# glennhickey/teHmm

Measured on AMD Instinct MI355X. Metric: genome positions/sec (Viterbi+posterior), 35 states x 10 tracks, higher is better.
Workload: dtype f64

## Files before the change

tehmm_amd/csrc/tehmm_fused.hip.h:

```cpp
#pragma once
#include "tehmm_lane.hip.h"

namespace tehmm {

template <int NT>
struct FusedGeom {
  static constexpr int KS = NT / 4;
  static constexpr int KSP = ((KS + 1) + 1) & ~1;
  static constexpr int RT = (NT + 15) / 16;
  static constexpr int SLICE_B = KSP * 8;
  static constexpr int ROW_D = 4 * KSP;
  static constexpr int ROW_D_LDS = 4 * KSP + 2;
};

#ifndef TEHMM_FUSED_2W
#define TEHMM_FUSED_2W 36
#endif
#define TEHMM_FUSED_BLKW 24
#ifndef TEHMM_FUSED_NSLOT_CAP
#define TEHMM_FUSED_NSLOT_CAP 64
#endif

struct FusedTab {
  const unsigned long long *rixx;
  const double *ptab;
  const double *ptab_lds;
  int FKW;
  int SB, NB;
  int K, n_glb;
  int lds_rows;
  double normalize;
};

template <int NT>
__device__ __forceinline__ void fused_load_lds(const double *lds, int row, int kq, double (&x)[FusedGeom<NT>::KSP]) {
  using G = FusedGeom<NT>;
  lds_cd2 *p = (lds_cd2 *)(size_t)((unsigned)(size_t)(__attribute__((address_space(3))) const double *)lds +
                                   (unsigned)(row * (G::ROW_D_LDS * 8) + kq * G::SLICE_B));
#pragma unroll
  for (int i = 0; i < G::KSP / 2; ++i) {
    const d2v v = p[i];
    x[2 * i] = v.x;
    x[2 * i + 1] = v.y;
  }
}
template <int NT>
__device__ __forceinline__ void fused_load_glb(const double *tab, int row, int kq, double (&x)[FusedGeom<NT>::KSP]) {
  using G = FusedGeom<NT>;
  const double2 *p = (const double2 *)(tab + ((int64_t)row * 4 + kq) * G::KSP);
#pragma unroll
  for (int i = 0; i < G::KSP / 2; ++i) {
    const double2 v = p[i];
    x[2 * i] = v.x;
    x[2 * i + 1] = v.y;
  }
}

__device__ __forceinline__ double item_sum4(double t) {
  const unsigned lo = __double2loint(t), hi = __double2hiint(t);
  const auto a = __builtin_amdgcn_permlane32_swap(lo, lo, false, false);
  const auto b = __builtin_amdgcn_permlane32_swap(hi, hi, false, false);
  const double t1 = __hiloint2double((int)b[0], (int)a[0]) + __hiloint2double((int)b[1], (int)a[1]);
  const unsigned lo1 = __double2loint(t1), hi1 = __double2hiint(t1);
  const auto c = __builtin_amdgcn_permlane16_swap(lo1, lo1, false, false);
  const auto d = __builtin_amdgcn_permlane16_swap(hi1, hi1, false, false);
  return __hiloint2double((int)d[0], (int)c[0]) + __hiloint2double((int)d[1], (int)c[1]);
}
__device__ __forceinline__ double item_max4(double t) {
  const unsigned lo = __double2loint(t), hi = __double2hiint(t);
  const auto a = __builtin_amdgcn_permlane32_swap(lo, lo, false, false);
  const auto b = __builtin_amdgcn_permlane32_swap(hi, hi, false, false);
  const double t1 = fmax(__hiloint2double((int)b[0], (int)a[0]), __hiloint2double((int)b[1], (int)a[1]));
  const unsigned lo1 = __double2loint(t1), hi1 = __double2hiint(t1);
  const auto c = __builtin_amdgcn_permlane16_swap(lo1, lo1, false, false);
  const auto d = __builtin_amdgcn_permlane16_swap(hi1, hi1, false, false);
  return fmax(__hiloint2double((int)d[0], (int)c[0]), __hiloint2double((int)d[1], (int)c[1]));
}

typedef unsigned int fused_u4 __attribute__((ext_vector_type(4)));
struct IndexWindow {
  const fused_u4 *src;
  unsigned lds_base;
  int lane, dir, NB;
  int cur = -1;
  fused_u4 r0, r1, r2;
  bool inflight = false;

  __device__ __forceinline__ void request(int blk) {
    if (blk < 0 || blk >= NB) { inflight = false; return; }
    const fused_u4 *p = src + (int64_t)blk * 192 + lane * 3;
    r0 = p[0];
    r1 = p[1];
    r2 = p[2];
    inflight = true;
  }
  __device__ __forceinline__ void commit(int blk) {
    typedef __attribute__((address_space(3))) fused_u4 lds_u4;
    lds_u4 *d = (lds_u4 *)(size_t)(lds_base + (unsigned)((blk & 1) * 3072 + lane * 48));
    d[0] = r0;
    d[1] = r1;
    d[2] = r2;
    cur = blk;
  }
  __device__ __forceinline__ void start(int blk) {
    request(blk);
    commit(blk);
    request(blk + dir);
  }
  __device__ __forceinline__ void need(int blk) {
    if (blk != cur) {
      commit(blk);
      request(blk + dir);
    }
  }
  __device__ __forceinline__ unsigned word_addr(int blk, int r, int FKW, int w) const {
    return lds_base + (unsigned)((blk & 1) * 3072 + ((r * FKW + w) * 16 + (lane & 15)) * 8);
  }
};
__device__ __forceinline__ unsigned long long lds_read_u64(unsigned addr) {
  typedef __attribute__((address_space(3))) const unsigned long long lds_cu64;
  return *(lds_cu64 *)(size_t)addr;
}

template <int NT, bool LOGDOM>
struct EmisStream {
  using G = FusedGeom<NT>;
  static constexpr int NSLOT = G::KS < TEHMM_FUSED_NSLOT_CAP ? G::KS : TEHMM_FUSED_NSLOT_CAP;
  static constexpr int NGS = NSLOT > 1 ? 2 : 1;
  static constexpr int GF = NSLOT >= 8 ? 4 : NSLOT / 2;
  const FusedTab &ft;
  const double *lds;
  IndexWindow &win;
  const int kq;
  unsigned wbase = 0;
  double q[G::KS];
  double sc = 0.0;
  double xa[G::KSP];
  double xc[G::KSP];
  unsigned long long wcur = 0;

  __device__ __forceinline__ EmisStream(const FusedTab &ft_, const double *lds_, IndexWindow &win_, int kq_)
      : ft(ft_), lds(lds_), win(win_), kq(kq_) {}
  static __device__ __forceinline__ int entry(unsigned long long w, int i) { return (int)((w >> (16 * (i & 3))) & 0xffffull); }
  __device__ __forceinline__ unsigned long long word(int w) const { return lds_read_u64(wbase + (unsigned)w * 128u); }
  __device__ __forceinline__ void fold(const double (&x)[G::KSP]) {
#pragma unroll
    for (int s = 0; s < G::KS; ++s) q[s] = LOGDOM ? q[s] + x[s] : q[s] * x[s];
    if (!LOGDOM) sc += x[G::KS];
  }
  __device__ __forceinline__ void glb_request(int i) { fused_load_glb<NT>(ft.ptab, entry(word(i >> 2), i), kq, xa); }
  __device__ __forceinline__ void begin(int e) {
    const int blk = e / ft.SB, r = e - blk * ft.SB;
    win.need(blk);
    wbase = win.word_addr(blk, r, ft.FKW, 0);
#pragma unroll
    for (int s = 0; s < G::KS; ++s) q[s] = LOGDOM ? 0.0 : 1.0;
    sc = 0.0;
    glb_request(0);
    wcur = word(ft.n_glb >> 2);
  }
  __device__ __forceinline__ void slot(int k) {
    if (k >= NSLOT) return;
    const int il = ft.n_glb + k;
    if (k > 0) fold(xc);
    if (k == GF && NSLOT > 1) {
      fold(xa);
      glb_request(1);
    }
    fused_load_lds<NT>(lds, entry(wcur, il), kq, xc);
    if (k + 1 < NSLOT) wcur = word((il + 1) >> 2);
  }
  __device__ __forceinline__ void finish(int N, double (&qo)[G::KS], double &ms) {
    fold(xc);
    fold(xa);
    for (int i = NGS; i < ft.n_glb; ++i) {
      glb_request(i);
      fold(xa);
    }
    for (int il = ft.n_glb + NSLOT; il < ft.K; ++il) {
      fused_load_lds<NT>(lds, entry(word(il >> 2), il), kq, xc);
      fold(xc);
    }
    if (LOGDOM) {
      double m = -INFINITY;
#pragma unroll
      for (int s = 0; s < G::KS; ++s) {
        q[s] *= ft.normalize;
        m = fmax(m, kq + 4 * s < N ? q[s] : -INFINITY);
      }
      m = item_max4(m);
      const bool good = m > -1e20;
#pragma unroll
      for (int s = 0; s < G::KS; ++s) qo[s] = (good && kq + 4 * s < N) ? exp_nonpos(q[s] - m) : 0.0;
      ms = good ? m : 0.0;
    } else {
#pragma unroll
      for (int s = 0; s < G::KS; ++s) qo[s] = q[s];
      ms = sc;
    }
  }
};

template <int NT>
__host__ __device__ inline size_t fused_lds_bytes(int lds_rows, bool post_tiles) {
  return (size_t)lds_rows * FusedGeom<NT>::ROW_D_LDS * 8 + 4 * 2 * 3072 + (post_tiles ? 4 * (16 * NT * 8 + 128) : 0);
}
template <int NT>
__device__ __forceinline__ void fused_stage(const FusedTab &ft, double *lds) {
  const int n = ft.lds_rows * FusedGeom<NT>::ROW_D_LDS;
  for (int i = threadIdx.x; i < n; i += blockDim.x) lds[i] = ft.ptab_lds[i];
}

struct FusedOrder {
  int K, n_glb, FKW, KP, SB, NB, Wu;
  int zero_glb, zero_lds;
  unsigned char order[TEHMM_MAX_TRACKS];
  int base[TEHMM_MAX_TRACKS];
  int cnt[TEHMM_MAX_TRACKS];
};
__global__ __launch_bounds__(256) void k_fused_rowindex(IntervalTab iv, LaneGeom lg, FusedOrder fo, const uint8_t *obs,
                                                        unsigned long long *rixx) {
  const int E = fo.NB * fo.SB;
  const int64_t n = (int64_t)lg.n_groups * 4 * E * 16;
  const int per_blk = 16 * fo.SB;
  for (int64_t idx = blockIdx.x * (int64_t)blockDim.x + threadIdx.x; idx < n; idx += (int64_t)gridDim.x * blockDim.x) {
    const int64_t tb = idx / per_blk;
    const int rem = (int)(idx - tb * per_blk);
    const int i16 = rem / fo.SB;
    const int e = (int)(tb % fo.NB) * fo.SB + (rem - i16 * fo.SB);
    const int64_t tile = tb / fo.NB;
    const int64_t item = tile * 16 + i16;
    const bool valid = item < lg.n_items;
    const int id = valid ? lg.item_iv[item] : 0;
    const int64_t T = iv.len[id];
    int64_t t = (valid ? lg.item_t0[item] : 0) - fo.Wu + e;
    t = t < 0 ? 0 : (t >= T ? T - 1 : t);
    const uint8_t *orow = obs + (iv.pos0[id] + (T > 0 ? t : 0)) * fo.KP;
    const int blk = e / fo.SB, r = e - blk * fo.SB;
    unsigned long long *dst = rixx + ((tile * fo.NB + blk) * TEHMM_FUSED_BLKW + (int64_t)r * fo.FKW) * 16 + i16;
    for (int w = 0; w < fo.FKW; ++w) {
      unsigned long long word = 0;
      for (int b = 0; b < 4; ++b) {
        const int i = 4 * w + b;
        int v = 0;
        if (i < fo.K) {
          const int sym = orow[fo.order[i]];
          v = sym < fo.cnt[i] ? fo.base[i] + sym : (i < fo.n_glb ? fo.zero_glb : fo.zero_lds);
        }
        word |= (unsigned long long)(v & 0xffff) << (16 * b);
      }
      dst[(int64_t)w * 16] = word;
    }
  }
}

template <int NT, bool LOGDOM>
__global__ __launch_bounds__(256) __attribute__((amdgpu_waves_per_eu(NT <= TEHMM_FUSED_2W ? 2 : 1, NT <= TEHMM_FUSED_2W ? 2 : 1)))
void k_fused_fwd(IntervalTab iv, FusedTab ft, LaneGeom lg, int N, int CS, int Wu,
                 const double *__restrict__ tab , float *al32, double *chkf, double *pre,
                 double *end, double *slog32) {
  using G = FusedGeom<NT>;
  constexpr int KS = G::KS, RT = G::RT;
  extern __shared__ double fused_lds[];
  fused_stage<NT>(ft, fused_lds);
  __syncthreads();
  const int lane = threadIdx.x & 63;
  const int tile = blockIdx.x * 4 + (threadIdx.x >> 6);
  if (tile >= lg.n_groups * 4) return;
  const int L = lg.L;
  const int kq = lane >> 4;
  const int64_t item = (int64_t)tile * 16 + (lane & 15);
  const bool valid = item < lg.n_items;
  const int id = valid ? lg.item_iv[item] : 0;
  const int64_t t0 = valid ? lg.item_t0[item] : 0;
  const int64_t T = iv.len[id];
  const int64_t ct0 = (t0 / CS) * CS;
  const bool run = valid && ct0 + CS <= T && ct0 > 0;
  if (!__any(run)) return;
  double tf[RT][KS];
#pragma unroll
  for (int rt = 0; rt < RT; ++rt) {
#pragma unroll
    for (int s = 0; s < KS; ++s) {
      const int j = 16 * rt + (lane & 15), k = 4 * s + kq;
      tf[rt][s] = (j < NT) ? tab[k * NT + j] : 0.0;
    }
  }
  double v[KS];
#pragma unroll
  for (int s = 0; s < KS; ++s) v[s] = (kq + 4 * s < N) ? 1.0 / (double)N : 0.0;
  double slog = 0.0;
  auto vec_out = [&](double *dst) {
    const int64_t po = ((((item >> 6) * NT) + kq) << 6) + (item & 63);
#pragma unroll
    for (int s = 0; s < KS; ++s) dst[po + ((int64_t)(4 * s) << 6)] = v[s];
  };
  const double qnan = __longlong_as_double(0x7ff8000000000000LL);
  IndexWindow win;
  win.src = (const fused_u4 *)ft.rixx + (int64_t)tile * ft.NB * 192;
  win.lds_base = (unsigned)(size_t)(__attribute__((address_space(3))) const double *)fused_lds +
                 (unsigned)(ft.lds_rows * G::ROW_D_LDS * 8 + (threadIdx.x >> 6) * 2 * 3072);
  win.lane = lane;
  win.dir = 1;
  win.NB = ft.NB;
  win.start(0);
  double q[KS], ms;
  EmisStream<NT, LOGDOM> es(ft, fused_lds, win, kq);
  es.begin(0);
#pragma unroll
  for (int k = 0; k < KS; ++k) es.slot(k);
  es.finish(N, q, ms);
  const int E1 = ft.NB * ft.SB - 1;
  es.begin(min(1, E1));
  {
    float2 *ar = (float2 *)al32 + al32_index<NT>(lg, item, 0, kq) / 2;
#pragma unroll
    for (int p = 0; p < (KS + 1) / 2; ++p) ar[(int64_t)p * 64] = make_float2(0.f, 0.f);
  }
#ifdef TEHMM_STAMPS
  unsigned long long stq[4] = {0, 0, 0, 0}, stt = stamp_now();
#define FST(i) do { const unsigned long long n_ = stamp_now(); stq[i] += n_ - stt; stt = n_; } while (0)
#else
#define FST(i)
#endif
  for (int s = -Wu; s < L; ++s) {
    if (s == 0) {
      if (run) vec_out(pre);
      slog = 0.0;
    }
    FST(3);
    lane_d4 acc[RT];
#pragma unroll
    for (int rt = 0; rt < RT; ++rt) acc[rt] = (lane_d4){0.0, 0.0, 0.0, 0.0};
#pragma unroll
    for (int k = 0; k < KS; ++k) {
#pragma unroll
      for (int rt = 0; rt < RT; ++rt) acc[rt] = __builtin_amdgcn_mfma_f64_16x16x4f64(tf[rt][k], v[k], acc[rt], 0, 0, 0);
      es.slot(k);
      __builtin_amdgcn_sched_barrier(0);
    }
    FST(0);
    double qn[KS], msn = 0.0;
    es.finish(N, qn, msn);
    FST(1);
    double a[KS];
    double t = 0.0;
#pragma unroll
    for (int k = 0; k < KS; ++k) {
      a[k] = acc[k >> 2][k & 3] * q[k];
      t += a[k];
    }
    t = item_sum4(t);
    const int e = ((__double2hiint(t) >> 20) & 0x7ff) - 1022;
    const bool okrow = t > 1e-280 && t < INFINITY;
    const double scale = okrow ? __hiloint2double((1023 - e) << 20, 0) : qnan;
#pragma unroll
    for (int k = 0; k < KS; ++k) v[k] = a[k] * scale;
    slog += (double)e * 0.6931471805599453 + ms;
#pragma unroll
    for (int k = 0; k < KS; ++k) q[k] = qn[k];
    const double ms_now = ms;
    ms = msn;
    (void)ms_now;
    es.begin(min(s + 2 + Wu, E1));
    FST(2);
    {
      float2 *ar = (float2 *)al32 + al32_index<NT>(lg, item, s < 0 ? 0 : s, kq) / 2;
#pragma unroll
      for (int p = 0; p < (KS + 1) / 2; ++p)
        ar[(int64_t)p * 64] = run ? make_float2((float)v[2 * p], 2 * p + 1 < KS ? (float)v[2 * p + 1] : 0.f)
                                  : make_float2(0.f, 0.f);
    }
    if (s >= 0 && run) {
      if ((s & 31) == 31) {
        if (kq == 0) slog32[item * (L / 32) + (s >> 5)] = slog;
        if ((s & 63) == 31) {
          double *cr = chkf + (item * (L / 64) + (s >> 6)) * NT + kq;
#pragma unroll
          for (int k = 0; k < KS; ++k) cr[4 * k] = v[k];
        }
      }
    }
  }
  if (run) vec_out(end);
#ifdef TEHMM_STAMPS
  if (lane == 0 && blockIdx.x < 4096)
    for (int i = 0; i < 4; ++i) g_stamps[(blockIdx.x * 4 + (threadIdx.x >> 6)) * 4 + i] = stq[i];
#endif
#undef FST
}

template <int NT, bool LOGDOM, bool EPS, bool ESTEP = false>
__global__ __launch_bounds__(256) __attribute__((amdgpu_waves_per_eu(NT <= TEHMM_FUSED_2W ? 2 : 1, NT <= TEHMM_FUSED_2W ? 2 : 1)))
void k_fused_bwd(IntervalTab iv, FusedTab ft, LaneGeom lg, int N, int CS, int Wu,
                 const double *__restrict__ tab , const float *__restrict__ al32,
                 double *post, double *pre, double *end, double *chk, float *gam32 = nullptr, float *wz32 = nullptr,
                 double *sink = nullptr ) {
  using G = FusedGeom<NT>;
  constexpr int KS = G::KS, RT = G::RT;
  extern __shared__ double fused_lds[];
  fused_stage<NT>(ft, fused_lds);
  __syncthreads();
  const int lane = threadIdx.x & 63;
  const int tile = blockIdx.x * 4 + (threadIdx.x >> 6);
  if (tile >= lg.n_groups * 4) return;
  const int L = lg.L;
  const int kq = lane >> 4;
  const int64_t item = (int64_t)tile * 16 + (lane & 15);
  const bool valid = item < lg.n_items;
  const int id = valid ? lg.item_iv[item] : 0;
  const int64_t t0 = valid ? lg.item_t0[item] : 0;
  const int64_t T = iv.len[id];
  const int64_t ct0 = (t0 / CS) * CS;
  const bool run = valid && ct0 + CS <= T && ct0 + CS < T;
  if (!__any(run)) return;
  const int wu = !run ? 0 : (int)min((int64_t)Wu, T - (t0 + L));
  double tf[RT][KS];
#pragma unroll
  for (int rt = 0; rt < RT; ++rt) {
#pragma unroll
    for (int s = 0; s < KS; ++s) {
      const int j = 16 * rt + (lane & 15), k = 4 * s + kq;
      tf[rt][s] = (j < NT) ? tab[j * NT + k] : 0.0;
    }
  }
  double v[KS];
#pragma unroll
  for (int s = 0; s < KS; ++s) v[s] = 0.0;
  const int64_t prow0 = (iv.out0[id] + t0) * N;
  auto vec_out = [&](double *dst) {
    const int64_t po = ((((item >> 6) * NT) + kq) << 6) + (item & 63);
#pragma unroll
    for (int s = 0; s < KS; ++s) dst[po + ((int64_t)(4 * s) << 6)] = v[s];
  };
  const double eps = 1.1920928955078125e-07;
  const double inv_epsden = 1.0 / (1.0 + (double)N * eps);
  const double qnan = __longlong_as_double(0x7ff8000000000000LL);
  const int top = L + wu - 1;
  IndexWindow win;
  win.src = (const fused_u4 *)ft.rixx + (int64_t)tile * ft.NB * 192;
  win.lds_base = (unsigned)(size_t)(__attribute__((address_space(3))) const double *)fused_lds +
                 (unsigned)(ft.lds_rows * G::ROW_D_LDS * 8 + (threadIdx.x >> 6) * 2 * 3072);
  win.lane = lane;
  win.dir = -1;
  win.NB = ft.NB;
  win.start((L + 2 * Wu - 1) / ft.SB);
  typedef __attribute__((address_space(3))) double lds_f64;
  typedef __attribute__((address_space(3))) long long lds_i64;
  const unsigned ptile = (unsigned)(size_t)(__attribute__((address_space(3))) const double *)fused_lds +
                         (unsigned)(ft.lds_rows * G::ROW_D_LDS * 8 + 4 * 2 * 3072 + (threadIdx.x >> 6) * (16 * NT * 8 + 128));
  const unsigned pinfo = ptile + 16 * NT * 8;
  if (!ESTEP && kq == 0) *(lds_i64 *)(size_t)(pinfo + (lane & 15) * 8) = run ? (long long)prow0 : -1ll;
  double q[KS], ms;
  EmisStream<NT, LOGDOM> es(ft, fused_lds, win, kq);
  es.begin(L + 2 * Wu - 1);
#pragma unroll
  for (int k = 0; k < KS; ++k) es.slot(k);
  es.finish(N, q, ms);
  es.begin(max(L + 2 * Wu - 2, 0));
#ifdef TEHMM_STAMPS
  unsigned long long stq[4] = {0, 0, 0, 0}, stt = stamp_now();
#define FST(i) do { const unsigned long long n_ = stamp_now(); stq[i] += n_ - stt; stt = n_; } while (0)
#else
#define FST(i)
#endif
  for (int s = L + Wu - 1; s >= 0; --s) {
    if (s == L - 1 && run) vec_out(pre);
    FST(3);
    lane_d4 acc[RT];
#pragma unroll
    for (int rt = 0; rt < RT; ++rt) acc[rt] = (lane_d4){0.0, 0.0, 0.0, 0.0};
    float2 alp[(KS + 1) / 2];
    {
      const float2 *ar = (const float2 *)al32 + al32_index<NT>(lg, item, s < L ? s : L - 1, kq) / 2;
#pragma unroll
      for (int p = 0; p < (KS + 1) / 2; ++p) alp[p] = ar[(int64_t)p * 64];
    }
#pragma unroll
    for (int k = 0; k < KS; ++k) {
#pragma unroll
      for (int rt = 0; rt < RT; ++rt) acc[rt] = __builtin_amdgcn_mfma_f64_16x16x4f64(tf[rt][k], v[k], acc[rt], 0, 0, 0);
      es.slot(k);
      __builtin_amdgcn_sched_barrier(0);
    }
    FST(0);
#pragma unroll
    for (int p = 0; p < (KS + 1) / 2; ++p) asm volatile("" : "+v"(alp[p].x), "+v"(alp[p].y));
#pragma unroll
    for (int p = 0; p < (KS + 1) / 2; ++p) alp[p] = run ? alp[p] : make_float2(0.f, 0.f);
    double qn[KS], msn = 0.0;
    es.finish(N, qn, msn);
    FST(1);
    double t = 0.0;
#pragma unroll
    for (int k = 0; k < KS; ++k) t += acc[k >> 2][k & 3];
    t = item_sum4(t);
    const int e = ((__double2hiint(t) >> 20) & 0x7ff) - 1022;
    double bt[KS];
    const bool okrow = (s >= L && s >= top) || (t > 0.0 && t < INFINITY);
    const double scale = okrow ? __hiloint2double((1023 - e) << 20, 0) : qnan;
#pragma unroll
    for (int k = 0; k < KS; ++k) {
      bt[k] = acc[k >> 2][k & 3] * scale;
      if (s >= L && s == top) bt[k] = kq + 4 * k < N ? 1.0 : 0.0;
    }
    double g[KS];
    float wzf[ESTEP ? KS : 1];
#pragma unroll
    for (int k = 0; k < KS; ++k) g[k] = 0.0;
#pragma unroll
    for (int k = 0; k < (ESTEP ? KS : 1); ++k) wzf[k] = 0.f;
    if (s < L) {
      double gt = 0.0;
#pragma unroll
      for (int k = 0; k < KS; ++k) {
        g[k] = (double)((k & 1) ? alp[k >> 1].y : alp[k >> 1].x) * bt[k];
        gt += g[k];
      }
      gt = item_sum4(gt);
      const double inv = 1.0 / gt;
#pragma unroll
      for (int k = 0; k < KS; ++k) {
        g[k] *= inv;
        if (EPS) g[k] = (g[k] + eps) * inv_epsden;
      }
      if constexpr (ESTEP) {
        const double wzs = scale * inv;
#pragma unroll
        for (int k = 0; k < KS; ++k) wzf[k] = (float)(v[k] * wzs);
      }
#pragma unroll
      for (int k = 0; k < KS; ++k) v[k] = q[k] * bt[k];
#pragma unroll
      for (int k = 0; k < KS; ++k) q[k] = qn[k];
    }
    if (s >= L) {
#pragma unroll
      for (int k = 0; k < KS; ++k) v[k] = s > top ? 0.0 : q[k] * bt[k];
#pragma unroll
      for (int k = 0; k < KS; ++k) q[k] = qn[k];
    }
    es.begin(max(s - 2 + Wu, 0));
    {
      const bool off = s < L;
      if constexpr (ESTEP) {
        const int64_t ai = al32_index<NT>(lg, item, off ? s : L - 1, kq) / 2;
        float2 *gr = (float2 *)gam32 + ai, *wr = (float2 *)wz32 + ai;
#pragma unroll
        for (int p = 0; p < (KS + 1) / 2; ++p) {
          gr[(int64_t)p * 64] = run ? make_float2((float)g[2 * p], 2 * p + 1 < KS ? (float)g[2 * p + 1] : 0.f)
                                    : make_float2(0.f, 0.f);
          wr[(int64_t)p * 64] = run ? make_float2(wzf[2 * p], 2 * p + 1 < KS ? wzf[2 * p + 1] : 0.f)
                                    : make_float2(0.f, 0.f);
        }
      } else {
#pragma unroll
        for (int k = 0; k < KS; ++k) *(lds_f64 *)(size_t)(ptile + (unsigned)(((lane & 15) * NT + kq + 4 * k) * 8)) = g[k];
        int lane_v = lane;
        asm volatile("" : "+v"(lane_v));
        double *const snk = sink + ((int64_t)tile << 6) + lane;
        int offv = off ? 1 : 0;
        asm volatile("" : "+v"(offv));
        constexpr int NJ = (16 * NT + 63) / 64;
        double val[NJ];
        long long rbase[NJ];
#pragma unroll
        for (int j = 0; j < NJ; ++j) {
          const int e = 64 * j + lane_v;
          const int ec = (16 * NT % 64 == 0 || e < 16 * NT) ? e : 0;
          const int r = (ec * (65536 / NT + 1)) >> 16;
          val[j] = *(lds_f64 *)(size_t)(ptile + (unsigned)ec * 8u);
          rbase[j] = *(lds_i64 *)(size_t)(pinfo + (unsigned)r * 8u);
        }
#pragma unroll
        for (int j = 0; j < NJ; ++j) {
          const int e = 64 * j + lane_v;
          const int ec = (16 * NT % 64 == 0 || e < 16 * NT) ? e : 0;
          const int r = (ec * (65536 / NT + 1)) >> 16, c = ec - r * NT;
          const bool real = (offv != 0) & (rbase[j] >= 0) & (c < N) & (16 * NT % 64 == 0 || e < 16 * NT);
          double *dst = real ? post + (rbase[j] + (int64_t)s * N + c) : snk;
          asm volatile("" : "+v"(dst));
          *(__attribute__((address_space(1))) double *)dst = val[j];
        }
      }
      if (off && run) {
        if ((s & 63) == 31) {
          double *cr = chk + (item * (L / 64) + (s >> 6)) * NT + kq;
#pragma unroll
          for (int k = 0; k < KS; ++k) cr[4 * k] = bt[k];
        }
      }
    }
    FST(2);
    ms = msn;
  }
  (void)ms;
  if (run) vec_out(end);
#ifdef TEHMM_STAMPS
  if (lane == 0 && blockIdx.x < 4096)
    for (int i = 0; i < 4; ++i) g_stamps[4096 * 16 + (blockIdx.x * 4 + (threadIdx.x >> 6)) * 4 + i] = stq[i];
#endif
#undef FST
}

}
```

tehmm_amd/csrc/tehmm_spec.hip.h:

```cpp
#pragma once
#include "tehmm_coop.hip.h"

namespace tehmm {

#define TEHMM_SPEC_NONE (-2147483647 - 1)
#ifndef TEHMM_SPEC_MIN_E
#define TEHMM_SPEC_MIN_E 15
#endif

struct VitChunks {
  const int *iv;
  const int64_t *t0;
  const int64_t *first;
  int n;
  int CS;
  const int *e;
  double *gain;
  int *ok;
  double *wmin;
  double *rows;
  int *ntie;
  int *ties;
  double *tierows;
  double *segmin;
// ... 509 lines not shown
  if (!__all(okl) || !(rmax > 0.0) || !(rmin < INFINITY)) return INFINITY;
  return rmax / rmin - 1.0;
}

template <int NT, int DIR>
__global__ __launch_bounds__(256) __attribute__((amdgpu_waves_per_eu(2, 2))) void k_fb_spec(IntervalTab iv, EmisTab em, FbChunks fc, int N,
                                                 const double *g_A, double *rows_out) {
  extern __shared__ double sm[];
  constexpr int RS = NT + 1;
  const int lane = threadIdx.x & 63;
  const int w = threadIdx.x >> 6;
  double *ring = sm + w * 64 * RS;
  double *ms = sm + 4 * 64 * RS + w * 64;
  const int jl = min(lane, NT - 1);
  const bool live = lane < N;
  double ac[NT];
#pragma unroll
  for (int i = 0; i < NT; ++i)
    ac[i] = live ? (DIR == 0 ? g_A[i * NT + jl] : g_A[jl * NT + i]) : (lane == NT - 1 ? 1.0 : 0.0);
  for (int c = blockIdx.x * 4 + w; c < fc.n; c += gridDim.x * 4) {
    const int id = fc.iv[c];
    const int64_t T = iv.len[id];
    const int64_t p0 = iv.pos0[id];
    const int64_t t0 = fc.t0[c];
    const int64_t t1 = t0 + fc.CS;
    if (t1 > T) continue;
    if (DIR == 0 && c == fc.first[id]) continue;
    if (DIR == 1 && t1 >= T) continue;
    double *out = rows_out + iv.out0[id] * N;
    double v = live ? 1.0 / (double)N : 0.0;
    double s = 0.0;
    bool seen = true;
    if (DIR == 1) {
      emis_block<NT, true, false, false>(em, nullptr, p0 + t1, 1, lane, N, seen, nullptr, nullptr, nullptr,
                                         ring, RS, ms);
      __builtin_amdgcn_wave_barrier();
      __builtin_amdgcn_s_waitcnt(0xc07f);
      v = live ? ring[jl] : 0.0;
      __builtin_amdgcn_wave_barrier();
    }
    for (int blk = 0; blk < fc.CS / 64; ++blk) {
      const int64_t lo = DIR == 0 ? t0 + 64 * blk : t1 - 64 * (blk + 1);
      if (DIR == 0)
        emis_block<NT, true, true, false>(em, nullptr, p0 + lo, 64, lane, N, seen, nullptr, nullptr, nullptr,
                                          ring, RS, ms);
      else
        emis_block<NT, true, false, false>(em, nullptr, p0 + lo, 64, lane, N, seen, nullptr, nullptr,
                                           nullptr, ring, RS, ms);
      __builtin_amdgcn_wave_barrier();
      __builtin_amdgcn_s_waitcnt(0xc07f);
      for (int q = 0; q < 64; ++q) {
        const int p = DIR == 0 ? q : 63 - q;
        const int64_t t = lo + p;
        const double bh = ring[p * RS + jl];
        double rr[(NT + 15) / 16];
        rep_rows<NT>(v, rr);
        double sacc[4] = {0.0, 0.0, 0.0, 0.0};
        asm volatile("s_nop 1" ::: "memory");
        BcastFma<0, NT>::run(rr, ac, sacc);
        const double ssum = (sacc[0] + sacc[1]) + (sacc[2] + sacc[3]);
        const int e = ((__builtin_amdgcn_readlane(__double2hiint(ssum), NT - 1) >> 20) & 0x7ff) - 1022;
        if (DIR == 0) {
          v = live ? ldexp(ssum * bh, -e) : 0.0;
          s += (double)e * 0.6931471805599453 + ms[p];
          if (live) out[t * N + lane] = v;
          if ((p & 31) == 31 && lane == 0) fc.scale[(int64_t)c * (fc.CS / 32) + (t - t0) / 32] = s;
        } else {
          const double bt = live ? ldexp(ssum, -e) : 0.0;
          if (live) out[t * N + lane] = bt;
          v = live ? bh * bt : 0.0;
          if (t == t0 && lane < NT) fc.wstart[(int64_t)c * NT + lane] = v;
        }
      }
      __builtin_amdgcn_wave_barrier();
    }
  }
}

template <int NT, int DIR>
__global__ __launch_bounds__(64) void k_fb_probe(IntervalTab iv, EmisTab em, int N, const double *g_A, const int *p_iv,
                                                 const int64_t *p_t0, int WMAX, int *steps) {
  extern __shared__ double sm[];
  constexpr int RS = NT + 1;
  const int lane = threadIdx.x & 63;
  double *ring = sm;
  double *ms = sm + 64 * RS;
  const int jl = min(lane, NT - 1);
  const bool live = lane < N;
  double ac[NT];
#pragma unroll
  for (int i = 0; i < NT; ++i)
    ac[i] = live ? (DIR == 0 ? g_A[i * NT + jl] : g_A[jl * NT + i]) : (lane == NT - 1 ? 1.0 : 0.0);
  const int id = p_iv[blockIdx.x];
  const int64_t p0 = iv.pos0[id];
  const int64_t t0 = p_t0[blockIdx.x];
  double u = live ? 1.0 / (double)N : 0.0;
  double v = live ? exp(-(double)lane) : 0.0;
  bool seen = true;
  int found = WMAX;
  for (int blk = 0; blk < WMAX / 64 && found == WMAX; ++blk) {
    const int64_t lo = DIR == 0 ? t0 + 64 * blk : t0 - 64 * (blk + 1);
    if (DIR == 0)
      emis_block<NT, true, true, false>(em, nullptr, p0 + lo, 64, lane, N, seen, nullptr, nullptr, nullptr, ring, RS, ms);
    else
      emis_block<NT, true, false, false>(em, nullptr, p0 + lo, 64, lane, N, seen, nullptr, nullptr, nullptr, ring, RS, ms);
    __builtin_amdgcn_wave_barrier();
    __builtin_amdgcn_s_waitcnt(0xc07f);
    for (int q = 0; q < 64; ++q) {
      const int p = DIR == 0 ? q : 63 - q;
      const double bh = ring[p * RS + jl];
      double x2[2] = {u, v};
#pragma unroll
      for (int c = 0; c < 2; ++c) {
        double rr[(NT + 15) / 16];
        rep_rows<NT>(x2[c], rr);
        double sacc[4] = {0.0, 0.0, 0.0, 0.0};
        asm volatile("s_nop 1" ::: "memory");
        BcastFma<0, NT>::run(rr, ac, sacc);
        const double ssum = (sacc[0] + sacc[1]) + (sacc[2] + sacc[3]);
        const int e = ((__builtin_amdgcn_readlane(__double2hiint(ssum), NT - 1) >> 20) & 0x7ff) - 1022;
        x2[c] = live ? ldexp(ssum * bh, -e) : 0.0;
      }
      u = x2[0];
      v = x2[1];
      double rho;
      const double d = proj_dist(u, v, live, rho);
      if (d <= 0.1 * TEHMM_FB_TOL || !(d == d)) {
        found = 64 * blk + q + 1;
        break;
      }
    }
    __builtin_amdgcn_wave_barrier();
  }
  if (lane == 0) steps[blockIdx.x] = found;
}

template <int NT, int DIR, bool TRATIO, bool LANE, bool FUSED = false, bool ESTEP = false>
__global__ __launch_bounds__(128) __attribute__((amdgpu_waves_per_eu(1, 1)))
void k_fb_fix(IntervalTab iv, EmisTab em, FbChunks fc, int N, const double *g_A, const double *g_lt,
              const double *g_pi, const double *tratios, double *rows, double *fwd_logprob,
              int *dead_flag, double *wrows, int *escale, int allow_jump, int *stats, LaneGeom lg,
              const int *okc, const double *chk = nullptr, double *post = nullptr, float *al32 = nullptr,
              const double *endv = nullptr, float *gam32 = nullptr, float *wz32 = nullptr) {
  extern __shared__ double sm[];
  constexpr int RS = NT + 1;
  constexpr int CPB = 64;
  double *ring = sm;
  double *msr = ring + 2 * CPB * RS;
  double *ltdv = msr + 2 * CPB;
  double *ltab = ltdv + NT;
  volatile int64_t *seqpos = (volatile int64_t *)(ltab + em.lds_rows * NT);
  volatile int *gen = (volatile int *)(seqpos + 4);
  double *wzu = (double *)(seqpos + 8);
  const int lane = threadIdx.x & 63;
  const int w = threadIdx.x >> 6;
  const int id = iv.order[blockIdx.x];
  const int64_t T = iv.len[id];
  const int64_t p0 = iv.pos0[id];
  if (T <= 0) return;
  const int jl = min(lane, NT - 1);
  const bool live = lane < N;
  if (threadIdx.x < NT) ltdv[threadIdx.x] = g_lt[threadIdx.x * NT + threadIdx.x];
  stage_emis_table(em, ltab, NT);
  const int64_t END = DIR == 0 ? T : 0;
  if (threadIdx.x == 0) {
    seqpos[0] = DIR == 0 ? 0 : T;
    seqpos[1] = seqpos[2] = seqpos[3] = END;
    *gen = 0;
  }
  const int64_t cfirst = fc.first[id];
  if (w == 0) __builtin_amdgcn_s_setprio(TEHMM_PRIO_HI);
  else __builtin_amdgcn_s_setprio(TEHMM_PRIO_LO);
  __syncthreads();
  bool seen = false;
  auto block_lo = [&](int64_t key) { return DIR == 0 ? key : ((key - 1) / CPB) * CPB; };
  auto block_np = [&](int64_t key) {
    return (int)(DIR == 0 ? min((int64_t)CPB, T - key) : key - ((key - 1) / CPB) * CPB);
  };
  auto done = [&](int64_t key) { return DIR == 0 ? key >= T : key <= 0; };
  auto emit = [&](int64_t key, int slot) {
    const int64_t lo = block_lo(key);
    const int np = block_np(key);
    if (DIR == 0)
      emis_block<NT, true, true, TRATIO>(em, ltab, p0 + lo, np, lane, N, seen, dead_flag + id, ltdv, tratios,
                                         ring + slot * CPB * RS, RS, msr + slot * CPB);
    else {
      bool dummy = true;
      emis_block<NT, true, false, TRATIO>(em, ltab, p0 + lo, np, lane, N, dummy, nullptr, ltdv, tratios,
                                          ring + slot * CPB * RS, RS, msr + slot * CPB);
    }
  };
  if (w == 1) emit(seqpos[0], 0);
  __syncthreads();
  if (w == 0) {
    double ac[NT];
#pragma unroll
    for (int i = 0; i < NT; ++i)
      ac[i] = live ? (DIR == 0 ? g_A[i * NT + jl] : g_A[jl * NT + i]) : (lane == NT - 1 ? 1.0 : 0.0);
    double *out = LANE ? rows : rows + iv.out0[id] * N;
    const int64_t ifirst = LANE ? lg.ifirst[id] : 0;
    auto rowp = [&](int64_t t) -> double * {
      if (LANE) return out + lane_row(lg, NT, ifirst + t / lg.L, t % lg.L) + ((int64_t)jl << 6);
      return out + t * N + lane;
    };
    int *es = (DIR == 0 && escale) ? escale + iv.out0[id] : nullptr;
    double *wr = (DIR == 1 && wrows) ? wrows + iv.out0[id] * N : nullptr;
    double Ecum = 0.0, Mcum = 0.0;
    double v = 0.0;
    int n_block = 0, n_jump = 0;
    for (int it = 0;; ++it) {
      const int64_t cur = seqpos[it & 3];
      if (done(cur)) break;
      if (it > (1 << 22)) { if (stats && lane == 0) atomicAdd(&stats[6], 1); break; }
      ++n_block;
      const int64_t lo = block_lo(cur);
      const int np = block_np(cur);
      const double *br = ring + (it & 1) * CPB * RS;
      const double *mr = msr + (it & 1) * CPB;
      const int64_t c = cfirst + lo / fc.CS;
      const int64_t ct0 = fc.t0[c];
      const bool cfull = ct0 + fc.CS <= T;
      const bool spec = allow_jump && np == CPB && cfull && (!LANE || okc[c] != 0) &&
                        (DIR == 0 ? (c != cfirst && lo + CPB < ct0 + fc.CS) : (ct0 + fc.CS < T && lo > ct0));
      double *brow = rowp(lo);
      const int64_t rstride = LANE ? (int64_t)NT << 6 : (int64_t)N;
      const int pg = DIR == 0 ? 31 : 32;
      const int64_t tg = DIR == 0 ? lo + pg : cur - 1 - pg;
      int64_t cj = c;
      if (LANE) {
        cj = DIR == 0 ? max(c, (int64_t)fc.runend_f[c]) : min(c, (int64_t)fc.runstart_b[c]);
        cj = DIR == 0 ? min(cj, (int64_t)fc.first[id + 1] - 1) : max(cj, cfirst);
      }
      const int64_t target = DIR == 0 ? fc.t0[cj] + fc.CS : fc.t0[cj];
      double srow = 0.0;
      if (spec) {
        if (FUSED)
          srow = live ? chk[((ifirst + tg / lg.L) * (lg.L / 64) + (tg % lg.L) / 64) * NT + jl] : 0.0;
        else
          srow = live ? brow[(tg - lo) * rstride] : 0.0;
      }
      else if (lane == 0) {
        seqpos[(it + 1) & 3] = DIR == 0 ? cur + np : lo;
        *gen = it + 1;
      }
      bool jump = false;
      double Sg = 0.0, rho = 1.0;
      for (int q = 0; q < np; ++q) {
        const int p = DIR == 0 ? q : np - 1 - q;
        const int64_t t = lo + p;
        const double bh = br[p * RS + jl];
        if (DIR == 0) {
          Mcum += mr[p];
          if (t == 0) {
            v = live ? exp(g_pi[jl]) * bh : 0.0;
          } else {
            double rr[(NT + 15) / 16];
            rep_rows<NT>(v, rr);
            double sacc[4] = {0.0, 0.0, 0.0, 0.0};
            asm volatile("s_nop 1" ::: "memory");
            BcastFma<0, NT>::run(rr, ac, sacc);
            const double ssum = (sacc[0] + sacc[1]) + (sacc[2] + sacc[3]);
            const int e = ((__builtin_amdgcn_readlane(__double2hiint(ssum), NT - 1) >> 20) & 0x7ff) - 1022;
            v = live ? ldexp(ssum * bh, -e) : 0.0;
            Ecum += (double)e;
            if (es && lane == 0) es[t] = e;
          }
          if (FUSED) {
            if (lane < NT) al32[al32_index<NT>(lg, ifirst + t / lg.L, t % lg.L, lane)] = live ? (float)v : 0.f;
          } else if (live) {
            brow[p * rstride] = v;
          }
        } else {
          double bt;
          if (t == T - 1) {
            bt = live ? 1.0 : 0.0;
            if (ESTEP && lane < NT) wzu[p * RS + lane] = 0.0;
          } else {
            double rr[(NT + 15) / 16];
            rep_rows<NT>(v, rr);
            double sacc[4] = {0.0, 0.0, 0.0, 0.0};
            asm volatile("s_nop 1" ::: "memory");
            BcastFma<0, NT>::run(rr, ac, sacc);
            const double ssum = (sacc[0] + sacc[1]) + (sacc[2] + sacc[3]);
            const int e = ((__builtin_amdgcn_readlane(__double2hiint(ssum), NT - 1) >> 20) & 0x7ff) - 1022;
            bt = live ? ldexp(ssum, -e) : 0.0;
            if (ESTEP && lane < NT) wzu[p * RS + lane] = live ? ldexp(v, -e) : 0.0;
          }
          if (FUSED) {
            if (lane < NT) const_cast<double *>(br)[p * RS + lane] = bt;
          } else if (live) {
            brow[p * rstride] = bt;
          }
          if (spec && q == pg) {
            const double d = proj_dist(bt, srow, live, rho);
            jump = d <= TEHMM_FB_TOL;
            if (lane == 0) { seqpos[(it + 1) & 3] = jump ? target : lo; *gen = it + 1; }
          }
          v = live ? bh * bt : 0.0;
          if (wr && live) wr[t * N + lane] = v;
        }
        if (DIR == 0 && spec && q == pg) {
          const double d = proj_dist(v, srow, live, rho);
          jump = d <= TEHMM_FB_TOL;
          Sg = Ecum * 0.6931471805599453 + Mcum;
          if (lane == 0) { seqpos[(it + 1) & 3] = jump ? target : cur + np; *gen = it + 1; }
        }
      }
      if (FUSED && DIR == 1 && ESTEP) {
        for (int p = 0; p < np; ++p) {
          const int64_t tp = lo + p;
          const int64_t ai = al32_index<NT>(lg, ifirst + tp / lg.L, tp % lg.L, jl);
          const double a = live ? (double)al32[ai] : 0.0;
          const double g = a * (live ? br[p * RS + lane] : 0.0);
          const double tot = wave_sum_f64(g);
          if (lane < NT) {
            gam32[ai] = live ? (float)(g / tot) : 0.f;
            wz32[ai] = live ? (float)(wzu[p * RS + lane] / tot) : 0.f;
          }
        }
      } else if (FUSED && DIR == 1) {
        const double eps = 1.1920928955078125e-07;
        const double inv_epsden = 1.0 / (1.0 + (double)N * eps);
        double *po = post + (iv.out0[id] + lo) * N;
        for (int p = 0; p < np; ++p) {
          const int64_t tp = lo + p;
          const double a = live ? (double)al32[al32_index<NT>(lg, ifirst + tp / lg.L, tp % lg.L, jl)] : 0.0;
          const double g = a * (live ? br[p * RS + lane] : 0.0);
          const double tot = wave_sum_f64(g);
          if (live) po[(int64_t)p * N + lane] = (g / tot + eps) * inv_epsden;
        }
      }
      if (jump) {
        ++n_jump;
        if (DIR == 0) {
          const int64_t tl = target - 1;
          if (FUSED) {
            const int64_t it_end = ifirst + tl / lg.L;
            v = live ? endv[((((it_end >> 6) * NT) + jl) << 6) + (it_end & 63)] : 0.0;
          } else {
            v = live ? *rowp(tl) : 0.0;
          }
          const double *sc = fc.scale + c * (fc.CS / 32);
          Mcum = Sg + log(rho) + (sc[fc.CS / 32 - 1] - sc[(tg - ct0) / 32]);
          if (LANE) Mcum += fc.pre_f[cj] - fc.pre_f[c];
          Ecum = 0.0;
        } else {
          v = live ? fc.wstart[cj * NT + jl] : 0.0;
        }
      }
      __syncthreads();
    }
    if (DIR == 0) {
      const double tot = wave_sum_f64(live ? v : 0.0);
      if (lane == 0) fwd_logprob[id] = log(tot) + Ecum * 0.6931471805599453 + Mcum;
    }
    if (stats && lane == 0) { atomicAdd(&stats[2 + 2 * DIR], n_block); atomicAdd(&stats[3 + 2 * DIR], n_jump); }
  } else {
    for (int it = 0;; ++it) {
      const int64_t cur = seqpos[it & 3];
      if (done(cur)) break;
      if (it > (1 << 22)) break;
      int spins = 0;
      while (*gen < it + 1) {
        __builtin_amdgcn_s_sleep(8);
        if (++spins > (1 << 26)) break;
      }
      const int64_t nx = seqpos[(it + 1) & 3];
      if (!done(nx)) emit(nx, (it + 1) & 1);
      __syncthreads();
    }
  }
}

}
```

Baseline: 1.531 billion.

## Split fused forward/backward loops into warmup and main phases with strength-reduced addressing

Splits the warmup and main time loops of the fused forward and backward kernels into two separately instantiated phases, so per-step branches on s disappear. It also replaces per-step index computation for al32, gam32 and post with pointer increments, with destination pointers and validity masks precomputed once before the main loop. It makes the tile index wave-uniform and swaps the exact reciprocal for an rcp plus one Newton step when the row is valid. The spec code gains an extra jump guard that checks end-vector finiteness, which touches correctness. The risks are more code size and register pressure from the duplicated loop bodies, and slightly different rounding from the approximate division.

After: 1.562 billion, median of 6. 2.0% higher.

```diff
diff --git a/tehmm_amd/csrc/tehmm_fused.hip.h b/tehmm_amd/csrc/tehmm_fused.hip.h
--- a/tehmm_amd/csrc/tehmm_fused.hip.h
+++ b/tehmm_amd/csrc/tehmm_fused.hip.h
@@ -1,4 +1,5 @@
 #pragma once
+#include <type_traits>
 #include "tehmm_lane.hip.h"
 
 namespace tehmm {
@@ -265,7 +266,7 @@
   fused_stage<NT>(ft, fused_lds);
   __syncthreads();
   const int lane = threadIdx.x & 63;
-  const int tile = blockIdx.x * 4 + (threadIdx.x >> 6);
+  const int tile = __builtin_amdgcn_readfirstlane(blockIdx.x * 4 + (threadIdx.x >> 6));
   if (tile >= lg.n_groups * 4) return;
   const int L = lg.L;
   const int kq = lane >> 4;
@@ -312,22 +313,16 @@
   es.finish(N, q, ms);
   const int E1 = ft.NB * ft.SB - 1;
   es.begin(min(1, E1));
-  {
-    float2 *ar = (float2 *)al32 + al32_index<NT>(lg, item, 0, kq) / 2;
-#pragma unroll
-    for (int p = 0; p < (KS + 1) / 2; ++p) ar[(int64_t)p * 64] = make_float2(0.f, 0.f);
-  }
 #ifdef TEHMM_STAMPS
   unsigned long long stq[4] = {0, 0, 0, 0}, stt = stamp_now();
 #define FST(i) do { const unsigned long long n_ = stamp_now(); stq[i] += n_ - stt; stt = n_; } while (0)
 #else
 #define FST(i)
 #endif
-  for (int s = -Wu; s < L; ++s) {
-    if (s == 0) {
-      if (run) vec_out(pre);
-      slog = 0.0;
-    }
+  float2 *ar = (float2 *)al32 + al32_index<NT>(lg, item, 0, kq) / 2;
+  const int64_t ar_step = (al32_index<NT>(lg, item, 1, kq) - al32_index<NT>(lg, item, 0, kq)) / 2;
+  auto step = [&](const int s, auto official) __attribute__((always_inline)) {
+    constexpr bool OFFICIAL = decltype(official)::value;
     FST(3);
     lane_d4 acc[RT];
 #pragma unroll
@@ -359,29 +354,35 @@
     slog += (double)e * 0.6931471805599453 + ms;
 #pragma unroll
     for (int k = 0; k < KS; ++k) q[k] = qn[k];
-    const double ms_now = ms;
     ms = msn;
-    (void)ms_now;
     es.begin(min(s + 2 + Wu, E1));
     FST(2);
-    {
-      float2 *ar = (float2 *)al32 + al32_index<NT>(lg, item, s < 0 ? 0 : s, kq) / 2;
+    if constexpr (OFFICIAL) {
 #pragma unroll
       for (int p = 0; p < (KS + 1) / 2; ++p)
         ar[(int64_t)p * 64] = run ? make_float2((float)v[2 * p], 2 * p + 1 < KS ? (float)v[2 * p + 1] : 0.f)
                                   : make_float2(0.f, 0.f);
-    }
-    if (s >= 0 && run) {
-      if ((s & 31) == 31) {
-        if (kq == 0) slog32[item * (L / 32) + (s >> 5)] = slog;
-        if ((s & 63) == 31) {
-          double *cr = chkf + (item * (L / 64) + (s >> 6)) * NT + kq;
-#pragma unroll
-          for (int k = 0; k < KS; ++k) cr[4 * k] = v[k];
+      ar += ar_step;
+      if (run) {
+        if ((s & 31) == 31) {
+          if (kq == 0) slog32[item * (L / 32) + (s >> 5)] = slog;
+          if ((s & 63) == 31) {
+            double *cr = chkf + (item * (L / 64) + (s >> 6)) * NT + kq;
+#pragma unroll
+            for (int k = 0; k < KS; ++k) cr[4 * k] = v[k];
+          }
         }
       }
     }
-  }
+  };
+  for (int s = -Wu; s < 0; ++s) step(s, std::false_type{});
+  {
+#pragma unroll
+    for (int p = 0; p < (KS + 1) / 2; ++p) ar[(int64_t)p * 64] = make_float2(0.f, 0.f);
+  }
+  if (run) vec_out(pre);
+  slog = 0.0;
+  for (int s = 0; s < L; ++s) step(s, std::true_type{});
   if (run) vec_out(end);
 #ifdef TEHMM_STAMPS
   if (lane == 0 && blockIdx.x < 4096)
@@ -402,7 +403,7 @@
   fused_stage<NT>(ft, fused_lds);
   __syncthreads();
   const int lane = threadIdx.x & 63;
-  const int tile = blockIdx.x * 4 + (threadIdx.x >> 6);
+  const int tile = __builtin_amdgcn_readfirstlane(blockIdx.x * 4 + (threadIdx.x >> 6));
   if (tile >= lg.n_groups * 4) return;
   const int L = lg.L;
   const int kq = lane >> 4;
@@ -451,6 +452,13 @@
                          (unsigned)(ft.lds_rows * G::ROW_D_LDS * 8 + 4 * 2 * 3072 + (threadIdx.x >> 6) * (16 * NT * 8 + 128));
   const unsigned pinfo = ptile + 16 * NT * 8;
   if (!ESTEP && kq == 0) *(lds_i64 *)(size_t)(pinfo + (lane & 15) * 8) = run ? (long long)prow0 : -1ll;
+  constexpr int NJ = ESTEP ? 1 : (16 * NT + 63) / 64;
+  double *pdst[NJ];
+  unsigned long long preal[NJ];
+  const int64_t ar_step = (al32_index<NT>(lg, item, 1, kq) - al32_index<NT>(lg, item, 0, kq)) / 2;
+  const int64_t ar_last = al32_index<NT>(lg, item, L - 1, kq) / 2;
+  const float2 *alr = (const float2 *)al32 + ar_last;
+  float2 *gr = ESTEP ? (float2 *)gam32 + ar_last : nullptr, *wr = ESTEP ? (float2 *)wz32 + ar_last : nullptr;
   double q[KS], ms;
   EmisStream<NT, LOGDOM> es(ft, fused_lds, win, kq);
   es.begin(L + 2 * Wu - 1);
@@ -464,17 +472,17 @@
 #else
 #define FST(i)
 #endif
-  for (int s = L + Wu - 1; s >= 0; --s) {
-    if (s == L - 1 && run) vec_out(pre);
+  auto step = [&](const int s, auto official) __attribute__((always_inline)) {
+    constexpr bool OFFICIAL = decltype(official)::value;
     FST(3);
     lane_d4 acc[RT];
 #pragma unroll
     for (int rt = 0; rt < RT; ++rt) acc[rt] = (lane_d4){0.0, 0.0, 0.0, 0.0};
     float2 alp[(KS + 1) / 2];
-    {
-      const float2 *ar = (const float2 *)al32 + al32_index<NT>(lg, item, s < L ? s : L - 1, kq) / 2;
-#pragma unroll
-      for (int p = 0; p < (KS + 1) / 2; ++p) alp[p] = ar[(int64_t)p * 64];
+    if constexpr (OFFICIAL) {
+#pragma unroll
+      for (int p = 0; p < (KS + 1) / 2; ++p) alp[p] = alr[(int64_t)p * 64];
+      alr -= ar_step;
     }
 #pragma unroll
     for (int k = 0; k < KS; ++k) {
@@ -484,10 +492,12 @@
       __builtin_amdgcn_sched_barrier(0);
     }
     FST(0);
-#pragma unroll
-    for (int p = 0; p < (KS + 1) / 2; ++p) asm volatile("" : "+v"(alp[p].x), "+v"(alp[p].y));
-#pragma unroll
-    for (int p = 0; p < (KS + 1) / 2; ++p) alp[p] = run ? alp[p] : make_float2(0.f, 0.f);
+    if constexpr (OFFICIAL) {
+#pragma unroll
+      for (int p = 0; p < (KS + 1) / 2; ++p) asm volatile("" : "+v"(alp[p].x), "+v"(alp[p].y));
+#pragma unroll
+      for (int p = 0; p < (KS + 1) / 2; ++p) alp[p] = run ? alp[p] : make_float2(0.f, 0.f);
+    }
     double qn[KS], msn = 0.0;
     es.finish(N, qn, msn);
     FST(1);
@@ -497,20 +507,22 @@
     t = item_sum4(t);
     const int e = ((__double2hiint(t) >> 20) & 0x7ff) - 1022;
     double bt[KS];
-    const bool okrow = (s >= L && s >= top) || (t > 0.0 && t < INFINITY);
+    const bool okrow = (!OFFICIAL && s >= top) || (t > 0.0 && t < INFINITY);
     const double scale = okrow ? __hiloint2double((1023 - e) << 20, 0) : qnan;
 #pragma unroll
     for (int k = 0; k < KS; ++k) {
       bt[k] = acc[k >> 2][k & 3] * scale;
-      if (s >= L && s == top) bt[k] = kq + 4 * k < N ? 1.0 : 0.0;
-    }
-    double g[KS];
-    float wzf[ESTEP ? KS : 1];
-#pragma unroll
-    for (int k = 0; k < KS; ++k) g[k] = 0.0;
-#pragma unroll
-    for (int k = 0; k < (ESTEP ? KS : 1); ++k) wzf[k] = 0.f;
-    if (s < L) {
+      if (!OFFICIAL && s == top) bt[k] = kq + 4 * k < N ? 1.0 : 0.0;
+    }
+    if constexpr (!OFFICIAL) {
+#pragma unroll
+      for (int k = 0; k < KS; ++k) v[k] = s > top ? 0.0 : q[k] * bt[k];
+#pragma unroll
+      for (int k = 0; k < KS; ++k) q[k] = qn[k];
+      es.begin(max(s - 2 + Wu, 0));
+    } else {
+      double g[KS];
+      float wzf[ESTEP ? KS : 1];
       double gt = 0.0;
 #pragma unroll
       for (int k = 0; k < KS; ++k) {
@@ -518,7 +530,18 @@
         gt += g[k];
       }
       gt = item_sum4(gt);
-      const double inv = 1.0 / gt;
+      double inv;
+#ifndef TEHMM_FUSED_EXACT_DIV
+      if (__builtin_expect(okrow, 1)) {
+        const double x = __builtin_amdgcn_rcp(gt);
+        inv = __builtin_fma(x, __builtin_fma(-gt, x, 1.0), x);
+      } else {
+        asm volatile("");
+        inv = 1.0 / gt;
+      }
+#else
+      inv = 1.0 / gt;
+#endif
 #pragma unroll
       for (int k = 0; k < KS; ++k) {
         g[k] *= inv;
@@ -533,19 +556,8 @@
       for (int k = 0; k < KS; ++k) v[k] = q[k] * bt[k];
 #pragma unroll
       for (int k = 0; k < KS; ++k) q[k] = qn[k];
-    }
-    if (s >= L) {
-#pragma unroll
-      for (int k = 0; k < KS; ++k) v[k] = s > top ? 0.0 : q[k] * bt[k];
-#pragma unroll
-      for (int k = 0; k < KS; ++k) q[k] = qn[k];
-    }
-    es.begin(max(s - 2 + Wu, 0));
-    {
-      const bool off = s < L;
+      es.begin(max(s - 2 + Wu, 0));
       if constexpr (ESTEP) {
-        const int64_t ai = al32_index<NT>(lg, item, off ? s : L - 1, kq) / 2;
-        float2 *gr = (float2 *)gam32 + ai, *wr = (float2 *)wz32 + ai;
 #pragma unroll
         for (int p = 0; p < (KS + 1) / 2; ++p) {
           gr[(int64_t)p * 64] = run ? make_float2((float)g[2 * p], 2 * p + 1 < KS ? (float)g[2 * p + 1] : 0.f)
@@ -553,37 +565,29 @@
           wr[(int64_t)p * 64] = run ? make_float2(wzf[2 * p], 2 * p + 1 < KS ? wzf[2 * p + 1] : 0.f)
                                     : make_float2(0.f, 0.f);
         }
+        gr -= ar_step;
+        wr -= ar_step;
       } else {
 #pragma unroll
         for (int k = 0; k < KS; ++k) *(lds_f64 *)(size_t)(ptile + (unsigned)(((lane & 15) * NT + kq + 4 * k) * 8)) = g[k];
-        int lane_v = lane;
-        asm volatile("" : "+v"(lane_v));
-        double *const snk = sink + ((int64_t)tile << 6) + lane;
-        int offv = off ? 1 : 0;
-        asm volatile("" : "+v"(offv));
-        constexpr int NJ = (16 * NT + 63) / 64;
         double val[NJ];
-        long long rbase[NJ];
 #pragma unroll
         for (int j = 0; j < NJ; ++j) {
-          const int e = 64 * j + lane_v;
+          const int e = 64 * j + lane;
           const int ec = (16 * NT % 64 == 0 || e < 16 * NT) ? e : 0;
-          const int r = (ec * (65536 / NT + 1)) >> 16;
           val[j] = *(lds_f64 *)(size_t)(ptile + (unsigned)ec * 8u);
-          rbase[j] = *(lds_i64 *)(size_t)(pinfo + (unsigned)r * 8u);
         }
+        unsigned n8 = (unsigned)N * 8u;
+        asm volatile("" : "+v"(n8));
 #pragma unroll
         for (int j = 0; j < NJ; ++j) {
-          const int e = 64 * j + lane_v;
-          const int ec = (16 * NT % 64 == 0 || e < 16 * NT) ? e : 0;
-          const int r = (ec * (65536 / NT + 1)) >> 16, c = ec - r * NT;
-          const bool real = (offv != 0) & (rbase[j] >= 0) & (c < N) & (16 * NT % 64 == 0 || e < 16 * NT);
-          double *dst = real ? post + (rbase[j] + (int64_t)s * N + c) : snk;
-          asm volatile("" : "+v"(dst));
-          *(__attribute__((address_space(1))) double *)dst = val[j];
+          *(__attribute__((address_space(1))) double *)pdst[j] = val[j];
+          unsigned dec;
+          asm("v_cndmask_b32_e64 %0, 0, %1, %2" : "=v"(dec) : "v"(n8), "s"(preal[j]));
+          pdst[j] = (double *)((char *)pdst[j] - dec);
         }
       }
-      if (off && run) {
+      if (run) {
         if ((s & 63) == 31) {
           double *cr = chk + (item * (L / 64) + (s >> 6)) * NT + kq;
 #pragma unroll
@@ -593,7 +597,24 @@
     }
     FST(2);
     ms = msn;
-  }
+  };
+  for (int s = L + Wu - 1; s >= L; --s) step(s, std::false_type{});
+  if (run) vec_out(pre);
+  if constexpr (!ESTEP) {
+    double *const snk = sink + ((int64_t)tile << 6) + lane;
+#pragma unroll
+    for (int j = 0; j < NJ; ++j) {
+      const int e = 64 * j + lane;
+      const bool inb = 16 * NT % 64 == 0 || e < 16 * NT;
+      const int ec = inb ? e : 0;
+      const int r = ec / NT, c = ec - r * NT;
+      const long long rb = *(lds_i64 *)(size_t)(pinfo + (unsigned)r * 8u);
+      const bool real = inb && rb >= 0 && c < N;
+      pdst[j] = real ? post + (rb + (int64_t)(L - 1) * N + c) : snk;
+      preal[j] = __builtin_amdgcn_ballot_w64(real);
+    }
+  }
+  for (int s = L - 1; s >= 0; --s) step(s, std::true_type{});
   (void)ms;
   if (run) vec_out(end);
 #ifdef TEHMM_STAMPS
diff --git a/tehmm_amd/csrc/tehmm_spec.hip.h b/tehmm_amd/csrc/tehmm_spec.hip.h
--- a/tehmm_amd/csrc/tehmm_spec.hip.h
+++ b/tehmm_amd/csrc/tehmm_spec.hip.h
@@ -835,6 +835,11 @@
         if (DIR == 0 && spec && q == pg) {
           const double d = proj_dist(v, srow, live, rho);
           jump = d <= TEHMM_FB_TOL;
+          if (FUSED) {
+            const int64_t it_end = ifirst + (target - 1) / lg.L;
+            const double ev = live ? endv[((((it_end >> 6) * NT) + jl) << 6) + (it_end & 63)] : 0.0;
+            jump = jump && __all(ev >= 0.0 && ev < INFINITY);
+          }
           Sg = Ecum * 0.6931471805599453 + Mcum;
           if (lane == 0) { seqpos[(it + 1) & 3] = jump ? target : cur + np; *gen = it + 1; }
         }
```
